# cp2k/dbcsr

Measured on AMD Instinct MI355X. Metric: block-sparse multiply GFLOP/s (fp64), higher is better.
Workload: dtype f64; 1 GPU; config2_32768_23x23_fill10_fp64; M=32768, c_nblks=2030625, nproducts=29207882, k_passes=1, parallelism=1 GPU

## Files before the change

dbcsr_amd/csrc/mm_exact.h:

```cpp
#ifndef DBCSR_AMD_MM_EXACT_H
#define DBCSR_AMD_MM_EXACT_H
#include "mm_types.h"
#include "smm_core.h"
#include "mm_epilogue.h"

#ifndef DBCSR_EXACT_ALL_PIECES
#define DBCSR_EXACT_ALL_PIECES 1
#endif
#ifndef DBCSR_EXACT_SCHED_BARRIER
#define DBCSR_EXACT_SCHED_BARRIER 1
#endif

namespace dbcsr_amd {

template <int LD>
struct Pitch {
  static constexpr int PAD = (LD % 16 == 0) ? 2 : 0;
  static constexpr int P = LD + PAD;
};

constexpr int cmax(int a, int b) { return a > b ? a : b; }
template <int V>
struct IntC {
  static constexpr int value = V;
};

constexpr int class_wave_lds(int m, int n, int k0, int k1, int k2) {
  int a_lds = 0, cb_max = 0, bpad = 0;
  const int ks[3] = {k0, k1, k2};
  for (int i = 0; i < 3; ++i) {
    const int k = ks[i];
    if (k <= 0) continue;
    const int k4 = 4 * ((k + 3) / 4), ap = m + ((m % 16 == 0) ? 2 : 0);
    a_lds = cmax(a_lds, ap * k4 * 8);
    cb_max = cmax(cb_max, (k * n * 8 + 1023) / 1024);
    if (k % 16 == 0) bpad = 128;
  }
  a_lds = (a_lds + 15) & ~15;
  const int c_lds = ((m * n * 8 + 1023) / 1024) * 1024;
  return (cmax(a_lds + cb_max * (1024 + bpad) + 16, c_lds) + 15) & ~15;
}

template <int M, int N, int K>
struct KShape {
  static constexpr int KS = (K + 3) / 4, K4 = 4 * KS;
  static constexpr int AP = Pitch<M>::P, BP = Pitch<K>::P;
  static constexpr int A_LDS = AP * K4 * 8, B_LDS = BP * N * 8;
  static constexpr int CA = (M * K4 * 8 + 1023) / 1024, CB = (K * N * 8 + 1023) / 1024;
};
template <int M, int N>
struct KShape<M, N, 0> {
  static constexpr int KS = 0, K4 = 0, AP = 0, BP = 0, A_LDS = 0, B_LDS = 0, CA = 0, CB = 0;
};

template <int M, int N, int K0, int K1, int K2>
struct ClassShape {
  static constexpr int MA = (M + 7) / 8, NC = (N + 7) / 8;
  static constexpr int A_LDS = (cmax(KShape<M, N, K0>::A_LDS, cmax(KShape<M, N, K1>::A_LDS, KShape<M, N, K2>::A_LDS)) + 15) & ~15;
  static constexpr int CAMAX = cmax(KShape<M, N, K0>::CA, cmax(KShape<M, N, K1>::CA, KShape<M, N, K2>::CA));
  static constexpr int CBMAX = cmax(KShape<M, N, K0>::CB, cmax(KShape<M, N, K1>::CB, KShape<M, N, K2>::CB));
  static constexpr int BPAD = ((K0 % 16 == 0) || (K1 != 0 && K1 % 16 == 0) || (K2 != 0 && K2 % 16 == 0)) ? 128 : 0;
  static constexpr int B_REGION = CBMAX * (1024 + BPAD) + 16;
  static constexpr int C_LDS = ((M * N * 8 + 1023) / 1024) * 1024;
  static constexpr int WAVE_LDS = (cmax(A_LDS + B_REGION, C_LDS) + 15) & ~15;
  static_assert(WAVE_LDS == class_wave_lds(M, N, K0, K1, K2), "host and device disagree on the LDS size of a class");
};

template <int LD>
__device__ __forceinline__ int staged_offset(int c, int lane) {
  if constexpr (Pitch<LD>::PAD == 0)
    return c * 1024 + lane * 16;
  else
    return c * 1024 + lane * 16 + Pitch<LD>::PAD * 8 * ((c * 128) / LD + (lane * 2) / LD);
}

template <int M, int N, int K0, int K1, int K2>
__device__ __forceinline__ void cblock_f64_classes(const Desc& d, const Entry first, bool have_first, const Entry* __restrict__ entries,
                                                   const double* __restrict__ a_data,
                                                   const double* __restrict__ b_data, double* __restrict__ c_out,
                                                   const double* __restrict__ c_in, double alpha, double beta, const LaneMap& L, int lane,
                                                   char* lds, double* __restrict__ norm_out, double drop_below = 0.0) {
  typedef ClassShape<M, N, K0, K1, K2> CS;
  constexpr int MA = CS::MA, NC = CS::NC;
  constexpr int AP = Pitch<M>::P;
  char* lds_a = lds;
  char* lds_b = lds + CS::A_LDS;
  double acc[MA][NC];
#pragma unroll
  for (int a = 0; a < MA; ++a)
#pragma unroll
    for (int c = 0; c < NC; ++c) acc[a][c] = 0.0;
  const Entry* e = entries + d.prod_start;
  const int cnt = d.prod_cnt;
  const int voff = lane * 16;
  u32x4 ra[CS::CAMAX], rb[CS::CBMAX];

  const double* pa[MA];
  int colc[NC];
#pragma unroll
  for (int a = 0; a < MA; ++a) {
    int row = 8 * a + L.rowl;
    row = row < M ? row : M - 1;
    pa[a] = reinterpret_cast<const double*>(lds_a) + row + AP * L.kq;
  }
#pragma unroll
  for (int c = 0; c < NC; ++c) {
    int col = 8 * c + L.coll;
    colc[c] = col < N ? col : N - 1;
  }

  int ebase = 0;
  uint32_t ev0 = 0, ev1 = 0, ev2 = 1;
  auto load_window = [&](int base) {
    ebase = base;
    if (cnt <= 0) return;
    const int i = base + lane < cnt ? base + lane : cnt - 1;
    ev0 = e[i].a_lo;
    ev1 = e[i].b_lo;
    ev2 = e[i].w;
  };
  load_window(0);
  auto entry_at = [&](int i) {
    if (i - ebase >= 64) load_window(i);
    const int j = __builtin_amdgcn_readfirstlane(i - ebase);
    Entry en;
    en.a_lo = (uint32_t)__builtin_amdgcn_readlane((int)ev0, j);
    en.b_lo = (uint32_t)__builtin_amdgcn_readlane((int)ev1, j);
    en.w = (uint32_t)__builtin_amdgcn_readlane((int)ev2, j);
    return en;
  };
  auto in_set = [](int ks) { return ks == K0 || (K1 != 0 && ks == K1) || (K2 != 0 && ks == K2); };
  auto next_in_set = [&](int i) {
    while (i < cnt && !in_set(entry_at(i).ks())) ++i;
    return i;
  };

  auto issue = [&](const Entry& en) {
    const int ks = en.ks();
    const int abytes = __builtin_amdgcn_readfirstlane(M * ks * 8), bbytes = __builtin_amdgcn_readfirstlane(ks * N * 8);
    const int nca = __builtin_amdgcn_readfirstlane((M * ((ks + 3) & ~3) * 8 + 1023) >> 10), ncb = (bbytes + 1023) >> 10;
    const __amdgpu_buffer_rsrc_t rsa = __builtin_amdgcn_make_buffer_rsrc((void*)(a_data + en.a_off()), 0, abytes, 0x00020000);
    const __amdgpu_buffer_rsrc_t rsb = __builtin_amdgcn_make_buffer_rsrc((void*)(b_data + en.b_off()), 0, bbytes, 0x00020000);
#pragma unroll
    for (int c = 0; c < CS::CAMAX; ++c)
      if (DBCSR_EXACT_ALL_PIECES || c < nca) ra[c] = __builtin_amdgcn_raw_buffer_load_b128(rsa, voff, c * 1024, 0);
#pragma unroll
    for (int c = 0; c < CS::CBMAX; ++c)
      if (DBCSR_EXACT_ALL_PIECES || c < ncb) rb[c] = __builtin_amdgcn_raw_buffer_load_b128(rsb, voff, c * 1024, 0);
  };
  auto store = [&](int ks) {
    const int nca = __builtin_amdgcn_readfirstlane((M * ((ks + 3) & ~3) * 8 + 1023) >> 10);
    const int ncb = __builtin_amdgcn_readfirstlane((ks * N * 8 + 1023) >> 10);
#pragma unroll
    for (int c = 0; c < CS::CAMAX; ++c)
      if (DBCSR_EXACT_ALL_PIECES || c < nca) *reinterpret_cast<u32x4*>(lds_a + staged_offset<M>(c, lane)) = ra[c];
    DBCSR_AMD_LDS_ORDER();
    const int sh = __builtin_amdgcn_readfirstlane((ks & 15) == 0 ? (ks == 16 ? 4 : 5) : 31);
#pragma unroll
    for (int c = 0; c < CS::CBMAX; ++c)
      if (DBCSR_EXACT_ALL_PIECES || c < ncb) *reinterpret_cast<u32x4*>(lds_b + c * 1024 + lane * 16 + 16 * ((c * 128 + lane * 2) >> sh)) = rb[c];
  };
  auto compute_k = [&](auto kc) {
    constexpr int K = decltype(kc)::value;
    typedef KShape<M, N, K> KSH;
    constexpr int KS = KSH::KS, BP = KSH::BP;
    const double* pb[NC];
    const double* pbt[NC];
#pragma unroll
    for (int c = 0; c < NC; ++c) {
      pb[c] = reinterpret_cast<const double*>(lds_b) + L.kq + BP * colc[c];
      const int kt = 4 * (KS - 1) + L.kq;
      pbt[c] = reinterpret_cast<const double*>(lds_b) + (kt < K ? kt : 0) + BP * colc[c];
    }
    const bool tail_in = 4 * (KS - 1) + L.kq < K;
    double av[2][MA], bv[2][NC];
    auto fetch = [&](int s, int buf) {
#pragma unroll
      for (int a = 0; a < MA; ++a) av[buf][a] = pa[a][s * 4 * AP];
#pragma unroll
      for (int c = 0; c < NC; ++c) bv[buf][c] = (s == KS - 1 && (K & 3)) ? (tail_in ? pbt[c][0] : 0.0) : pb[c][4 * s];
    };
    fetch(0, 0);
#pragma unroll
    for (int s = 0; s < KS; ++s) {
      if (s + 1 < KS) fetch(s + 1, (s + 1) & 1);
#pragma unroll
      for (int a = 0; a < MA; ++a)
#pragma unroll
        for (int c = 0; c < NC; ++c) acc[a][c] = __builtin_amdgcn_mfma_f64_4x4x4f64(av[s & 1][a], bv[s & 1][c], acc[a][c], 0, 0, 0);
      if (DBCSR_EXACT_SCHED_BARRIER) __builtin_amdgcn_sched_barrier(0);
    }
  };

  int i0;
  Entry e0;
  if (have_first && in_set(first.ks())) {
    i0 = 0;
    e0 = first;
    issue(e0);
  } else {
    i0 = next_in_set(0);
    e0 = i0 < cnt ? entry_at(i0) : Entry::make(0, 0, K0);
    if (i0 < cnt) issue(e0);
  }
  while (i0 < cnt) {
    const int kcur = e0.ks();
    const int i1 = next_in_set(i0 + 1);
    const Entry e1 = i1 < cnt ? entry_at(i1) : e0;
    store(kcur);
    if (i1 < cnt) issue(e1);
    if (kcur == K0) compute_k(IntC<K0>());
    if constexpr (K1 != 0)
      if (kcur == K1) compute_k(IntC<K1>());
    if constexpr (K2 != 0)
      if (kcur == K2) compute_k(IntC<K2>());
    i0 = i1;
    e0 = e1;
  }
  for (int p = 0; p < cnt; ++p) {
    const Entry ep = e[p];
    if (!in_set(ep.ks())) block_product_f64<MA, NC, false>(acc, a_data + ep.a_off(), b_data + ep.b_off(), M, N, ep.ks(), L);
  }

  const bool has_in = d.cin_off >= 0;
  if (norm_out && drop_below > 0.0 && !has_in) {
    const double s2 = acc_norm2<M, N>(acc, alpha, L);
    if (lane == 0) *norm_out = s2;
    if (s2 < drop_below) return;
    norm_out = nullptr;
  }
  stage_c_block<M, N>(reinterpret_cast<double*>(lds), acc, alpha, L);
  store_c_block<M, N>(lds, c_out + d.c_off, has_in ? c_in + d.cin_off : nullptr, beta, lane, norm_out);
}

template <int M, int N, int K0, int K1, int K2>
__device__ __forceinline__ void mm_class_kernel_body(const Desc* __restrict__ descs, int64_t nblk, const Entry* __restrict__ entries,
                                                     const double* __restrict__ a_data, const double* __restrict__ b_data,
                                                     double* __restrict__ c_out, const double* __restrict__ c_in, double alpha, double beta,
                                                     int skip_empty, const int* __restrict__ order, const Work* __restrict__ work,
                                                     double* __restrict__ norms, char* smem) {
  const int lane = threadIdx.x & 63;
  const int wid = __builtin_amdgcn_readfirstlane((int)(threadIdx.x >> 6));
  const int wg = xcd_remap(blockIdx.x, gridDim.x);
  const int64_t pos = (int64_t)wg * (int)(blockDim.x >> 6) + wid;
  Desc d;
  Entry first = Entry::make(0, 0, 0);
  bool have_first = false;
  int64_t cbi = 0;
  if (work) {
    const Work w = work[pos];
    if (w.prod_cnt < 0) return;
    cbi = w.cb;
    d.c_off = w.c_off, d.cin_off = w.cin_off, d.prod_start = w.prod_start, d.prod_cnt = w.prod_cnt, d.m = w.m, d.n = w.n;
    first.a_lo = w.a_lo, first.b_lo = w.b_lo, first.w = w.w;
    have_first = w.prod_cnt > 0;
  } else {
    const int64_t cb = order[pos];
    if (cb < 0 || cb >= nblk) return;
    d = descs[cb];
    cbi = cb;
  }
  const double drop_below = norms ? norms[nblk] : 0.0;
  if (skip_empty && d.prod_cnt == 0) return;
  const LaneMap L(lane);
  cblock_f64_classes<M, N, K0, K1, K2>(d, first, have_first, entries, a_data, b_data, c_out, c_in, alpha, beta, L, lane,
                                       smem + (size_t)wid * ClassShape<M, N, K0, K1, K2>::WAVE_LDS, norms ? norms + cbi : nullptr, drop_below);
}


template <int M, int N, int K0, int K1, int K2, int G>
__device__ __forceinline__ void mm_class_stream_body(const Desc* __restrict__ descs, int64_t nblk, const Entry* __restrict__ entries,
                                                     const double* __restrict__ a_data, const double* __restrict__ b_data,
                                                     double* __restrict__ c_out, const double* __restrict__ c_in, double alpha, double beta,
                                                     int skip_empty, const int* __restrict__ order, char* smem) {
  static_assert(G >= 1 && G <= 64, "one lane per block of the group");
  typedef ClassShape<M, N, K0, K1, K2> CS;
  constexpr int MA = CS::MA, NC = CS::NC;
  constexpr int AP = Pitch<M>::P;
  const int lane = threadIdx.x & 63;
  const int wid = __builtin_amdgcn_readfirstlane((int)(threadIdx.x >> 6));
  const int wg = xcd_remap(blockIdx.x, gridDim.x);
  const int64_t pos0 = ((int64_t)wg * 4 + wid) * G;
  char* lds = smem + (size_t)wid * CS::WAVE_LDS;
  char* lds_a = lds;
  char* lds_b = lds + CS::A_LDS;
  const LaneMap L(lane);
  const int voff = lane * 16;

  const int my_cb = lane < G ? order[pos0 + lane] : -1;
  const bool my_ok = my_cb >= 0 && my_cb < nblk;
  const Desc my_d = descs[my_ok ? my_cb : 0];
  const int my_cnt = my_ok ? my_d.prod_cnt : -1;
  auto lane_i32 = [&](int v, int l) { return __builtin_amdgcn_readlane(v, l); };
  auto lane_i64 = [&](int64_t v, int l) {
    const uint32_t lo = (uint32_t)__builtin_amdgcn_readlane((int)(uint32_t)v, l);
    const uint32_t hi = (uint32_t)__builtin_amdgcn_readlane((int)(uint32_t)((uint64_t)v >> 32), l);
    return (int64_t)(((uint64_t)hi << 32) | lo);
  };

  const double* pa[MA];
  int colc[NC];
#pragma unroll
  for (int a = 0; a < MA; ++a) {
    int row = 8 * a + L.rowl;
    row = row < M ? row : M - 1;
    pa[a] = reinterpret_cast<const double*>(lds_a) + row + AP * L.kq;
  }
#pragma unroll
  for (int c = 0; c < NC; ++c) {
    int col = 8 * c + L.coll;
    colc[c] = col < N ? col : N - 1;
  }
  u32x4 ra[CS::CAMAX], rb[CS::CBMAX];
  double acc[MA][NC];

  uint32_t w0[2] = {0, 0}, w1[2] = {0, 0}, w2[2] = {1, 1};
  auto load_window = [&](int buf, int b) {
    const int cnt = lane_i32(my_cnt, b);
    if (cnt <= 0) return;
    const Entry* e = entries + lane_i64(my_d.prod_start, b);
    const int i = lane < cnt ? lane : cnt - 1;
    const uint32_t x0 = e[i].a_lo, x1 = e[i].b_lo, x2 = e[i].w;
    if (buf) {
      w0[1] = x0, w1[1] = x1, w2[1] = x2;
    } else {
      w0[0] = x0, w1[0] = x1, w2[0] = x2;
    }
  };
  auto entry_at = [&](int buf, int b, int i) {
    Entry en;
    if (i < 64) {
      en.a_lo = (uint32_t)__builtin_amdgcn_readlane((int)(buf ? w0[1] : w0[0]), i);
      en.b_lo = (uint32_t)__builtin_amdgcn_readlane((int)(buf ? w1[1] : w1[0]), i);
      en.w = (uint32_t)__builtin_amdgcn_readlane((int)(buf ? w2[1] : w2[0]), i);
    } else {
      en = entries[lane_i64(my_d.prod_start, b) + i];
    }
    return en;
  };
  auto in_set = [](int ks) { return ks == K0 || (K1 != 0 && ks == K1) || (K2 != 0 && ks == K2); };

  auto issue = [&](const Entry& en) {
    const int ks = en.ks();
    const int abytes = __builtin_amdgcn_readfirstlane(M * ks * 8), bbytes = __builtin_amdgcn_readfirstlane(ks * N * 8);
    const __amdgpu_buffer_rsrc_t rsa = __builtin_amdgcn_make_buffer_rsrc((void*)(a_data + en.a_off()), 0, abytes, 0x00020000);
    const __amdgpu_buffer_rsrc_t rsb = __builtin_amdgcn_make_buffer_rsrc((void*)(b_data + en.b_off()), 0, bbytes, 0x00020000);
#pragma unroll
    for (int c = 0; c < CS::CAMAX; ++c) ra[c] = __builtin_amdgcn_raw_buffer_load_b128(rsa, voff, c * 1024, 0);
#pragma unroll
    for (int c = 0; c < CS::CBMAX; ++c) rb[c] = __builtin_amdgcn_raw_buffer_load_b128(rsb, voff, c * 1024, 0);
  };
  auto store = [&](int ks) {
#pragma unroll
    for (int c = 0; c < CS::CAMAX; ++c) *reinterpret_cast<u32x4*>(lds_a + staged_offset<M>(c, lane)) = ra[c];
    DBCSR_AMD_LDS_ORDER();
    const int sh = __builtin_amdgcn_readfirstlane((ks & 15) == 0 ? (ks == 16 ? 4 : 5) : 31);
#pragma unroll
    for (int c = 0; c < CS::CBMAX; ++c) *reinterpret_cast<u32x4*>(lds_b + c * 1024 + lane * 16 + 16 * ((c * 128 + lane * 2) >> sh)) = rb[c];
  };
  auto compute_k = [&](auto kc) {
    constexpr int K = decltype(kc)::value;
    typedef KShape<M, N, K> KSH;
    constexpr int KS = KSH::KS, BP = KSH::BP;
    const double* pb[NC];
    const double* pbt[NC];
#pragma unroll
    for (int c = 0; c < NC; ++c) {
      pb[c] = reinterpret_cast<const double*>(lds_b) + L.kq + BP * colc[c];
      const int kt = 4 * (KS - 1) + L.kq;
      pbt[c] = reinterpret_cast<const double*>(lds_b) + (kt < K ? kt : 0) + BP * colc[c];
    }
    const bool tail_in = 4 * (KS - 1) + L.kq < K;
    double av[2][MA], bv[2][NC];
    auto fetch = [&](int s, int buf) {
#pragma unroll
      for (int a = 0; a < MA; ++a) av[buf][a] = pa[a][s * 4 * AP];
#pragma unroll
      for (int c = 0; c < NC; ++c) bv[buf][c] = (s == KS - 1 && (K & 3)) ? (tail_in ? pbt[c][0] : 0.0) : pb[c][4 * s];
    };
    fetch(0, 0);
#pragma unroll
    for (int s = 0; s < KS; ++s) {
      if (s + 1 < KS) fetch(s + 1, (s + 1) & 1);
#pragma unroll
      for (int a = 0; a < MA; ++a)
#pragma unroll
        for (int c = 0; c < NC; ++c) acc[a][c] = __builtin_amdgcn_mfma_f64_4x4x4f64(av[s & 1][a], bv[s & 1][c], acc[a][c], 0, 0, 0);
      if (DBCSR_EXACT_SCHED_BARRIER) __builtin_amdgcn_sched_barrier(0);
    }
  };

  auto block_cnt = [&](int b) { return b < G ? lane_i32(my_cnt, b) : -1; };
  auto first_in_set = [&](int buf, int b, int from) {
    const int cnt = block_cnt(b);
    int i = from;
    while (i < cnt && !in_set(entry_at(buf, b, i).ks())) ++i;
    return i < cnt ? i : -1;
  };

  load_window(0, 0);
  int nb = 0, ni = first_in_set(0, 0, 0);
  bool in_flight = false;
  Entry ne = Entry::make(0, 0, K0);
  if (ni >= 0) {
    ne = entry_at(0, 0, ni);
    issue(ne);
    in_flight = true;
  }
  for (int b = 0; b < G; ++b) {
    const int buf = b & 1;
    const int cnt = block_cnt(b);
    if (b + 1 < G) load_window(buf ^ 1, b + 1);
    if (cnt < 0 || (skip_empty && cnt == 0)) {
      if (!in_flight && b + 1 < G) {
        ni = first_in_set(buf ^ 1, b + 1, 0);
        nb = b + 1;
        if (ni >= 0) {
          ne = entry_at(buf ^ 1, b + 1, ni);
          issue(ne);
          in_flight = true;
        }
      }
      continue;
    }
#pragma unroll
    for (int a = 0; a < MA; ++a)
#pragma unroll
      for (int c = 0; c < NC; ++c) acc[a][c] = 0.0;
    while (in_flight && nb == b) {
      const int kcur = ne.ks();
      store(kcur);
      int i1 = first_in_set(buf, b, ni + 1);
      in_flight = false;
      if (i1 >= 0) {
        ni = i1;
        ne = entry_at(buf, b, i1);
        issue(ne);
        in_flight = true;
      } else if (b + 1 < G) {
        i1 = first_in_set(buf ^ 1, b + 1, 0);
        nb = b + 1;
        ni = i1;
        if (i1 >= 0) {
          ne = entry_at(buf ^ 1, b + 1, i1);
          issue(ne);
          in_flight = true;
        }
      }
      if (kcur == K0) compute_k(IntC<K0>());
      if constexpr (K1 != 0)
        if (kcur == K1) compute_k(IntC<K1>());
      if constexpr (K2 != 0)
        if (kcur == K2) compute_k(IntC<K2>());
    }
    if (!in_flight && nb <= b && b + 1 < G) {
      ni = first_in_set(buf ^ 1, b + 1, 0);
      nb = b + 1;
      if (ni >= 0) {
        ne = entry_at(buf ^ 1, b + 1, ni);
        issue(ne);
        in_flight = true;
      }
    }
    const int64_t d_c_off = lane_i64(my_d.c_off, b), d_cin_off = lane_i64(my_d.cin_off, b), d_ps = lane_i64(my_d.prod_start, b);
    for (int p = 0; p < cnt; ++p) {
      const Entry ep = entries[d_ps + p];
      if (!in_set(ep.ks())) block_product_f64<MA, NC, false>(acc, a_data + ep.a_off(), b_data + ep.b_off(), M, N, ep.ks(), L);
    }
    stage_c_block<M, N>(reinterpret_cast<double*>(lds), acc, alpha, L);
    store_c_block<M, N>(lds, c_out + d_c_off, d_cin_off >= 0 ? c_in + d_cin_off : nullptr, beta, lane, nullptr);
  }
}

}

#ifdef DBCSR_AMD_JIT_M
#ifndef DBCSR_AMD_JIT_MINW
#define DBCSR_AMD_JIT_MINW 1
#endif
extern "C" __global__ void __launch_bounds__(256, DBCSR_AMD_JIT_MINW)
    mm_numeric_f64_class(const dbcsr_amd::Desc* __restrict__ descs, long nblk, const dbcsr_amd::Entry* __restrict__ entries,
                         const double* __restrict__ a_data, const double* __restrict__ b_data, double* __restrict__ c_out,
                         const double* __restrict__ c_in, double alpha, double beta, int skip_empty, const int* __restrict__ order,
                         const dbcsr_amd::Work* __restrict__ work, double* __restrict__ norms) {
  extern __shared__ __attribute__((aligned(16))) char smem[];
#if defined(DBCSR_AMD_JIT_G) && DBCSR_AMD_JIT_G > 1
  dbcsr_amd::mm_class_stream_body<DBCSR_AMD_JIT_M, DBCSR_AMD_JIT_N, DBCSR_AMD_JIT_K0, DBCSR_AMD_JIT_K1, DBCSR_AMD_JIT_K2, DBCSR_AMD_JIT_G>(
      descs, nblk, entries, a_data, b_data, c_out, c_in, alpha, beta, skip_empty, order, smem);
#else
  dbcsr_amd::mm_class_kernel_body<DBCSR_AMD_JIT_M, DBCSR_AMD_JIT_N, DBCSR_AMD_JIT_K0, DBCSR_AMD_JIT_K1, DBCSR_AMD_JIT_K2>(
      descs, nblk, entries, a_data, b_data, c_out, c_in, alpha, beta, skip_empty, order, work, norms, smem);
#endif
}
#endif
#endif
```

dbcsr_amd/csrc/mm_jit.hip:

```cpp
#include "mm_jit.h"

#include <dlfcn.h>
#include <unistd.h>
#include <cstdint>

#include <cstdio>
#include <cstdlib>
#include <cstring>
#include <map>
#include <mutex>
#include <string>
#include <tuple>
#include <vector>

#include "mm_exact.h"
#include "smm_exact.h"

namespace dbcsr_amd {
namespace {

#include "jit_sources.inc"

typedef struct _hiprtcProgram* rtc_program;
struct Rtc {
  void* lib = nullptr;
  int (*CreateProgram)(rtc_program*, const char*, const char*, int, const char**, const char**) = nullptr;
  int (*CompileProgram)(rtc_program, int, const char**) = nullptr;
  int (*GetProgramLogSize)(rtc_program, size_t*) = nullptr;
  int (*GetProgramLog)(rtc_program, char*) = nullptr;
  int (*GetCodeSize)(rtc_program, size_t*) = nullptr;
  int (*GetCode)(rtc_program, char*) = nullptr;
  int (*DestroyProgram)(rtc_program*) = nullptr;
  int (*Version)(int*, int*) = nullptr;
  bool ok = false;
};

Rtc& rtc() {
  static Rtc r;
  static std::once_flag once;
  std::call_once(once, [] {
    for (const char* name : {"libhiprtc.so", "libhiprtc.so.7", "/opt/rocm/lib/libhiprtc.so"}) {
      r.lib = dlopen(name, RTLD_NOW | RTLD_GLOBAL);
      if (r.lib) break;
    }
    if (!r.lib) {
      fprintf(stderr, "dbcsr_amd: cannot load libhiprtc (%s): mixed block sizes run the generic kernels\n", dlerror());
      return;
    }
#define DBCSR_SYM(field, sym)                               \
  *reinterpret_cast<void**>(&r.field) = dlsym(r.lib, sym);  \
  if (!r.field) return;
    DBCSR_SYM(CreateProgram, "hiprtcCreateProgram")
    DBCSR_SYM(CompileProgram, "hiprtcCompileProgram")
    DBCSR_SYM(GetProgramLogSize, "hiprtcGetProgramLogSize")
    DBCSR_SYM(GetProgramLog, "hiprtcGetProgramLog")
    DBCSR_SYM(GetCodeSize, "hiprtcGetCodeSize")
    DBCSR_SYM(GetCode, "hiprtcGetCode")
    DBCSR_SYM(DestroyProgram, "hiprtcDestroyProgram")
#undef DBCSR_SYM
    *reinterpret_cast<void**>(&r.Version) = dlsym(r.lib, "hiprtcVersion");
    r.ok = true;
  });
  return r;
}

struct Cached {
  std::vector<char> image;
  hipModule_t mod = nullptr;
  ClassKernel k;
  bool failed = false;
};
std::mutex g_mu;
std::map<std::tuple<int, int, int, int, int, int, int>, Cached> g_cache;

bool g_last_from_cache = false;
int compile_and_load(const char* defs, const char* tu_name, const char* what, const char* entry, const hipDeviceProp_t& prop, hipModule_t* mod,
                     hipFunction_t* fn, size_t* code_size, std::vector<char>* image) {
  Rtc& r = rtc();
  if (!r.ok) return -1;
  g_last_from_cache = false;
  const char* hsrc[] = {kJitSrc_mm_types, kJitSrc_smm_core, kJitSrc_mm_epilogue, kJitSrc_mm_exact, kJitSrc_smm_exact};
  const char* hname[] = {"mm_types.h", "smm_core.h", "mm_epilogue.h", "mm_exact.h", "smm_exact.h"};
  rtc_program prog = nullptr;
  if (r.CreateProgram(&prog, defs, tu_name, (int)(sizeof hname / sizeof hname[0]), hsrc, hname) != 0) return -1;
  std::string arch = std::string("--offload-arch=") + prop.gcnArchName;
  std::vector<std::string> extra;
  if (const char* d = getenv("DBCSR_AMD_JIT_DEFS")) {
    std::string all(d);
    size_t pos = 0;
    while (pos < all.size()) {
      const size_t e = all.find(' ', pos);
      const std::string tok = all.substr(pos, e == std::string::npos ? std::string::npos : e - pos);
      if (!tok.empty()) extra.push_back(tok);
      if (e == std::string::npos) break;
      pos = e + 1;
    }
  }
  std::vector<const char*> opts = {arch.c_str(), "-O3", "-std=c++17", "-munsafe-fp-atomics"};
  for (const std::string& t : extra) opts.push_back(t.c_str());
  std::string cache_file;
  if (const char* dir = getenv("DBCSR_AMD_JIT_CACHE")) {
    if (*dir) {
      uint64_t h = 1469598103934665603ull;
      auto mix = [&h](const char* t) {
        for (; *t; ++t) h = (h ^ (unsigned char)*t) * 1099511628211ull;
        h = (h ^ 0xffu) * 1099511628211ull;
      };
      mix(defs);
      for (const char* t : hsrc) mix(t);
      for (const char* t : opts) mix(t);
      int vmaj = 0, vmin = 0;
      if (r.Version) r.Version(&vmaj, &vmin);
      char tail[64];
      snprintf(tail, sizeof tail, "hiprtc %d.%d entry %s", vmaj, vmin, entry);
      mix(tail);
      char name[40];
      snprintf(name, sizeof name, "/dbcsr_amd_%016llx.co", (unsigned long long)h);
      cache_file = std::string(dir) + name;
      if (FILE* f = fopen(cache_file.c_str(), "rb")) {
        std::vector<char>& code = *image;
        code.clear();
        char buf[65536];
        size_t got;
        while ((got = fread(buf, 1, sizeof buf, f)) > 0) code.insert(code.end(), buf, buf + got);
        fclose(f);
        bool sound = false;
        if (code.size() > 24) {
          uint64_t head[3];
          memcpy(head, code.data(), 24);
          if (head[0] == 0x314f435f444d4143ull && head[1] == code.size() - 24) {
            uint64_t ph = 1469598103934665603ull;
            for (size_t i = 24; i < code.size(); ++i) ph = (ph ^ (unsigned char)code[i]) * 1099511628211ull;
            sound = ph == head[2];
          }
        }
        if (sound) code.erase(code.begin(), code.begin() + 24);
        if (sound && hipModuleLoadData(mod, code.data()) == hipSuccess) {
          if (hipModuleGetFunction(fn, *mod, entry) == hipSuccess) {
            r.DestroyProgram(&prog);
            if (code_size) *code_size = code.size();
            g_last_from_cache = true;
            if (getenv("DBCSR_AMD_MM_VERBOSE")) fprintf(stderr, "dbcsr_amd: %s from %s\n", what, cache_file.c_str());
            return 0;
          }
          (void)hipModuleUnload(*mod);
        }
        (void)hipGetLastError();
      }
    }
  }
  const int rc = r.CompileProgram(prog, (int)opts.size(), opts.data());
  if (rc != 0) {
    size_t ls = 0;
    r.GetProgramLogSize(prog, &ls);
    std::string log(ls + 1, 0);
    if (ls) r.GetProgramLog(prog, &log[0]);
    fprintf(stderr, "dbcsr_amd: hiprtc failed for %s:\n%s\n", what, log.c_str());
    r.DestroyProgram(&prog);
    return -1;
  }
  size_t cs = 0;
  r.GetCodeSize(prog, &cs);
  std::vector<char>& code = *image;
  code.assign(cs, 0);
  r.GetCode(prog, code.data());
  r.DestroyProgram(&prog);
  if (!cache_file.empty()) {
    const std::string tmp = cache_file + "." + std::to_string((long)getpid()) + ".tmp";
    if (FILE* f = fopen(tmp.c_str(), "wb")) {
      uint64_t head[3] = {0x314f435f444d4143ull, (uint64_t)code.size(), 1469598103934665603ull};
      for (char ch : code) head[2] = (head[2] ^ (unsigned char)ch) * 1099511628211ull;
      const bool ok = fwrite(head, 1, 24, f) == 24 && fwrite(code.data(), 1, code.size(), f) == code.size();
      if (fclose(f) != 0 || !ok || rename(tmp.c_str(), cache_file.c_str()) != 0) remove(tmp.c_str());
    }
  }
  if (hipModuleLoadData(mod, code.data()) != hipSuccess) return -1;
  if (hipModuleGetFunction(fn, *mod, entry) != hipSuccess) return -1;
  if (code_size) *code_size = cs;
  return 0;
}

struct CachedStack {
  std::vector<char> image;
  hipModule_t mod = nullptr;
  StackKernel k;
  bool failed = false;
};
std::map<std::tuple<int, int, int, int, int>, CachedStack> g_stack_cache;

}

int jit_class_kernel(int m, int n, int k0, int k1, int k2, int g, ClassKernel* out) {
  if (g < 1 || g > 64) return -1;
  if (!out || m < 1 || n < 1 || k0 < 1 || m > 32 || n > 32 || k0 > 32 || k1 > 32 || k2 > 32) return -1;
  int dev = 0;
  if (hipGetDevice(&dev) != hipSuccess) return -1;
  std::lock_guard<std::mutex> lock(g_mu);
  auto key = std::make_tuple(dev, m, n, k0, k1, k2, g);
  auto it = g_cache.find(key);
  if (it != g_cache.end()) {
    if (it->second.failed) return -1;
    *out = it->second.k;
    return 0;
  }
  Cached& c = g_cache[key];
  c.failed = true;
  hipDeviceProp_t prop;
  if (hipGetDeviceProperties(&prop, dev) != hipSuccess) return -1;
  const int wave_lds = class_wave_lds(m, n, k0, k1, k2);
  int wgs = (160 * 1024) / (4 * wave_lds);
  int minw = wgs > 4 ? 4 : (wgs < 1 ? 1 : wgs);
  if (g > 1 && minw > 1) --minw;
  char defs[512];
  snprintf(defs, sizeof defs,
           "#define DBCSR_AMD_JIT_M %d\n#define DBCSR_AMD_JIT_N %d\n#define DBCSR_AMD_JIT_K0 %d\n#define DBCSR_AMD_JIT_K1 %d\n"
           "#define DBCSR_AMD_JIT_K2 %d\n#define DBCSR_AMD_JIT_MINW %d\n#define DBCSR_AMD_JIT_G %d\n#include \"mm_exact.h\"\n",
           m, n, k0, k1, k2, minw, g);
  char what[96];
  snprintf(what, sizeof what, "class (%d, %d; %d, %d, %d)", m, n, k0, k1, k2);
  size_t cs = 0;
  if (compile_and_load(defs, "mm_class.hip", what, "mm_numeric_f64_class", prop, &c.mod, &c.k.fn, &cs, &c.image) != 0) return -1;
  c.k.wave_lds = wave_lds;
  c.failed = false;
  if (getenv("DBCSR_AMD_MM_VERBOSE") && !g_last_from_cache) fprintf(stderr, "dbcsr_amd: compiled class kernel (%d, %d; %d, %d, %d), %zu bytes, %d B LDS per wave\n", m, n, k0, k1, k2, cs, wave_lds);
  *out = c.k;
  return 0;
}


int jit_stack_kernel(int m, int n, int k, bool bt, StackKernel* out, bool compile) {
  if (!out || m < 1 || n < 1 || k < 1 || m > 32 || n > 32 || k > 32) return -1;
  int dev = 0;
  if (hipGetDevice(&dev) != hipSuccess) return -1;
  std::lock_guard<std::mutex> lock(g_mu);
  auto key = std::make_tuple(dev, m, n, k, (int)bt);
  auto it = g_stack_cache.find(key);
  if (it != g_stack_cache.end()) {
    if (it->second.failed) return -1;
    *out = it->second.k;
    return 0;
  }
  if (!compile) return 1;
  CachedStack& c = g_stack_cache[key];
  c.failed = true;
  hipDeviceProp_t prop;
  if (hipGetDeviceProperties(&prop, dev) != hipSuccess) return -1;
  const int wave_lds = stack_wave_lds(m, n, k, bt);
  int wgs = (160 * 1024) / (4 * wave_lds);
  const int minw = wgs > 4 ? 4 : (wgs < 1 ? 1 : wgs);
  char defs[512];
  snprintf(defs, sizeof defs,
           "#define DBCSR_AMD_JIT_SM %d\n#define DBCSR_AMD_JIT_SN %d\n#define DBCSR_AMD_JIT_SK %d\n#define DBCSR_AMD_JIT_SBT %d\n"
           "#define DBCSR_AMD_JIT_MINW %d\n#include \"smm_exact.h\"\n",
           m, n, k, bt ? 1 : 0, minw);
  char what[96];
  snprintf(what, sizeof what, "stack kernel (%d, %d, %d%s)", m, n, k, bt ? "; B transposed" : "");
  size_t cs = 0;
  if (compile_and_load(defs, "smm_stack_exact.hip", what, "smm_stack_f64_exact", prop, &c.mod, &c.k.fn, &cs, &c.image) != 0) return -1;
  c.k.wave_lds = wave_lds;
  c.failed = false;
  if (getenv("DBCSR_AMD_MM_VERBOSE") && !g_last_from_cache) fprintf(stderr, "dbcsr_amd: compiled %s, %zu bytes, %d B LDS per wave\n", what, cs, wave_lds);
  *out = c.k;
  return 0;
}

}
```

Baseline: 37360 GFLOP/s.

## Shrink per-wave LDS to the exact B image and guard staging stores

The per-wave LDS budget for each class now uses the padded B image size instead of whole 1 KiB pieces plus pad. Smaller LDS per wave allows more waves per CU. Staging stores are now skipped for pieces past the real A/B image, and are masked per lane when a piece would run past the smaller region. The JIT cache key now includes DBCSR_AMD_JIT_DEFS. The shared LDS-size helper moves into its own header that is also passed to the JIT compiler. The risk is extra branching in the store path and possible LDS overlap if the bounds logic is wrong.

```diff
diff --git a/dbcsr_amd/csrc/mm_class_lds.h b/dbcsr_amd/csrc/mm_class_lds.h
--- /dev/null
+++ b/dbcsr_amd/csrc/mm_class_lds.h
@@ -0,0 +1,24 @@
+#ifndef DBCSR_AMD_MM_CLASS_LDS_H
+#define DBCSR_AMD_MM_CLASS_LDS_H
+
+namespace dbcsr_amd {
+
+constexpr int cmax(int a, int b) { return a > b ? a : b; }
+
+constexpr int class_wave_lds(int m, int n, int k0, int k1, int k2) {
+  int a_lds = 0, b_lds = 0;
+  const int ks[3] = {k0, k1, k2};
+  for (int i = 0; i < 3; ++i) {
+    const int k = ks[i];
+    if (k <= 0) continue;
+    const int k4 = 4 * ((k + 3) / 4), ap = m + ((m % 16 == 0) ? 2 : 0), bp = k + ((k % 16 == 0) ? 2 : 0);
+    a_lds = cmax(a_lds, ap * k4 * 8);
+    b_lds = cmax(b_lds, (bp * n * 8 + 15) & ~15);
+  }
+  a_lds = (a_lds + 15) & ~15;
+  const int c_lds = ((m * n * 8 + 1023) / 1024) * 1024;
+  return (cmax(a_lds + b_lds, c_lds) + 15) & ~15;
+}
+
+}
+#endif
diff --git a/dbcsr_amd/csrc/mm_exact.h b/dbcsr_amd/csrc/mm_exact.h
--- a/dbcsr_amd/csrc/mm_exact.h
+++ b/dbcsr_amd/csrc/mm_exact.h
@@ -3,6 +3,7 @@
 #include "mm_types.h"
 #include "smm_core.h"
 #include "mm_epilogue.h"
+#include "mm_class_lds.h"
 
 #ifndef DBCSR_EXACT_ALL_PIECES
 #define DBCSR_EXACT_ALL_PIECES 1
@@ -19,33 +20,16 @@
   static constexpr int P = LD + PAD;
 };
 
-constexpr int cmax(int a, int b) { return a > b ? a : b; }
 template <int V>
 struct IntC {
   static constexpr int value = V;
 };
 
-constexpr int class_wave_lds(int m, int n, int k0, int k1, int k2) {
-  int a_lds = 0, cb_max = 0, bpad = 0;
-  const int ks[3] = {k0, k1, k2};
-  for (int i = 0; i < 3; ++i) {
-    const int k = ks[i];
-    if (k <= 0) continue;
-    const int k4 = 4 * ((k + 3) / 4), ap = m + ((m % 16 == 0) ? 2 : 0);
-    a_lds = cmax(a_lds, ap * k4 * 8);
-    cb_max = cmax(cb_max, (k * n * 8 + 1023) / 1024);
-    if (k % 16 == 0) bpad = 128;
-  }
-  a_lds = (a_lds + 15) & ~15;
-  const int c_lds = ((m * n * 8 + 1023) / 1024) * 1024;
-  return (cmax(a_lds + cb_max * (1024 + bpad) + 16, c_lds) + 15) & ~15;
-}
-
 template <int M, int N, int K>
 struct KShape {
   static constexpr int KS = (K + 3) / 4, K4 = 4 * KS;
   static constexpr int AP = Pitch<M>::P, BP = Pitch<K>::P;
-  static constexpr int A_LDS = AP * K4 * 8, B_LDS = BP * N * 8;
+  static constexpr int A_LDS = AP * K4 * 8, B_LDS = (BP * N * 8 + 15) & ~15;
   static constexpr int CA = (M * K4 * 8 + 1023) / 1024, CB = (K * N * 8 + 1023) / 1024;
 };
 template <int M, int N>
@@ -59,11 +43,13 @@
   static constexpr int A_LDS = (cmax(KShape<M, N, K0>::A_LDS, cmax(KShape<M, N, K1>::A_LDS, KShape<M, N, K2>::A_LDS)) + 15) & ~15;
   static constexpr int CAMAX = cmax(KShape<M, N, K0>::CA, cmax(KShape<M, N, K1>::CA, KShape<M, N, K2>::CA));
   static constexpr int CBMAX = cmax(KShape<M, N, K0>::CB, cmax(KShape<M, N, K1>::CB, KShape<M, N, K2>::CB));
-  static constexpr int BPAD = ((K0 % 16 == 0) || (K1 != 0 && K1 % 16 == 0) || (K2 != 0 && K2 % 16 == 0)) ? 128 : 0;
-  static constexpr int B_REGION = CBMAX * (1024 + BPAD) + 16;
+  static constexpr int B_LDS = cmax(KShape<M, N, K0>::B_LDS, cmax(KShape<M, N, K1>::B_LDS, KShape<M, N, K2>::B_LDS));
   static constexpr int C_LDS = ((M * N * 8 + 1023) / 1024) * 1024;
-  static constexpr int WAVE_LDS = (cmax(A_LDS + B_REGION, C_LDS) + 15) & ~15;
+  static constexpr int WAVE_LDS = (cmax(A_LDS + B_LDS, C_LDS) + 15) & ~15;
   static_assert(WAVE_LDS == class_wave_lds(M, N, K0, K1, K2), "host and device disagree on the LDS size of a class");
+  static constexpr bool B_PADDED = (K0 % 16 == 0) || (K1 != 0 && K1 % 16 == 0) || (K2 != 0 && K2 % 16 == 0);
+  static constexpr bool a_piece_passes(int c) { return c * 1024 + 1024 + (Pitch<M>::PAD ? 16 * ((c * 128 + 126) / M) : 0) > WAVE_LDS; }
+  static constexpr bool b_piece_passes(int c) { return A_LDS + c * 1024 + 1024 + (B_PADDED ? 16 * ((c * 128 + 126) / 16) : 0) > WAVE_LDS; }
 };
 
 template <int LD>
@@ -72,6 +58,25 @@
     return c * 1024 + lane * 16;
   else
     return c * 1024 + lane * 16 + Pitch<LD>::PAD * 8 * ((c * 128) / LD + (lane * 2) / LD);
+}
+
+template <class CS, int M, int N>
+__device__ __forceinline__ void stage_pieces(char* lds_a, char* lds_b, const u32x4 (&ra)[CS::CAMAX], const u32x4 (&rb)[CS::CBMAX], int ks, int lane) {
+  const int voff = lane * 16;
+  const int aimg = __builtin_amdgcn_readfirstlane(M * ((ks + 3) & ~3) * 8), bimg = __builtin_amdgcn_readfirstlane(ks * N * 8);
+#pragma unroll
+  for (int c = 0; c < CS::CAMAX; ++c)
+    if (c * 1024 < aimg) {
+      if (!CS::a_piece_passes(c) || c * 1024 + voff < aimg) *reinterpret_cast<u32x4*>(lds_a + staged_offset<M>(c, lane)) = ra[c];
+    }
+  DBCSR_AMD_LDS_ORDER();
+  const int sh = __builtin_amdgcn_readfirstlane((ks & 15) == 0 ? (ks == 16 ? 4 : 5) : 31);
+#pragma unroll
+  for (int c = 0; c < CS::CBMAX; ++c)
+    if (c * 1024 < bimg) {
+      if (!CS::b_piece_passes(c) || c * 1024 + voff < bimg)
+        *reinterpret_cast<u32x4*>(lds_b + c * 1024 + lane * 16 + 16 * ((c * 128 + lane * 2) >> sh)) = rb[c];
+    }
 }
 
 template <int M, int N, int K0, int K1, int K2>
@@ -148,18 +153,7 @@
     for (int c = 0; c < CS::CBMAX; ++c)
       if (DBCSR_EXACT_ALL_PIECES || c < ncb) rb[c] = __builtin_amdgcn_raw_buffer_load_b128(rsb, voff, c * 1024, 0);
   };
-  auto store = [&](int ks) {
-    const int nca = __builtin_amdgcn_readfirstlane((M * ((ks + 3) & ~3) * 8 + 1023) >> 10);
-    const int ncb = __builtin_amdgcn_readfirstlane((ks * N * 8 + 1023) >> 10);
-#pragma unroll
-    for (int c = 0; c < CS::CAMAX; ++c)
-      if (DBCSR_EXACT_ALL_PIECES || c < nca) *reinterpret_cast<u32x4*>(lds_a + staged_offset<M>(c, lane)) = ra[c];
-    DBCSR_AMD_LDS_ORDER();
-    const int sh = __builtin_amdgcn_readfirstlane((ks & 15) == 0 ? (ks == 16 ? 4 : 5) : 31);
-#pragma unroll
-    for (int c = 0; c < CS::CBMAX; ++c)
-      if (DBCSR_EXACT_ALL_PIECES || c < ncb) *reinterpret_cast<u32x4*>(lds_b + c * 1024 + lane * 16 + 16 * ((c * 128 + lane * 2) >> sh)) = rb[c];
-  };
+  auto store = [&](int ks) { stage_pieces<CS, M, N>(lds_a, lds_b, ra, rb, ks, lane); };
   auto compute_k = [&](auto kc) {
     constexpr int K = decltype(kc)::value;
     typedef KShape<M, N, K> KSH;
@@ -350,14 +344,7 @@
 #pragma unroll
     for (int c = 0; c < CS::CBMAX; ++c) rb[c] = __builtin_amdgcn_raw_buffer_load_b128(rsb, voff, c * 1024, 0);
   };
-  auto store = [&](int ks) {
-#pragma unroll
-    for (int c = 0; c < CS::CAMAX; ++c) *reinterpret_cast<u32x4*>(lds_a + staged_offset<M>(c, lane)) = ra[c];
-    DBCSR_AMD_LDS_ORDER();
-    const int sh = __builtin_amdgcn_readfirstlane((ks & 15) == 0 ? (ks == 16 ? 4 : 5) : 31);
-#pragma unroll
-    for (int c = 0; c < CS::CBMAX; ++c) *reinterpret_cast<u32x4*>(lds_b + c * 1024 + lane * 16 + 16 * ((c * 128 + lane * 2) >> sh)) = rb[c];
-  };
+  auto store = [&](int ks) { stage_pieces<CS, M, N>(lds_a, lds_b, ra, rb, ks, lane); };
   auto compute_k = [&](auto kc) {
     constexpr int K = decltype(kc)::value;
     typedef KShape<M, N, K> KSH;
diff --git a/dbcsr_amd/csrc/mm_jit.hip b/dbcsr_amd/csrc/mm_jit.hip
--- a/dbcsr_amd/csrc/mm_jit.hip
+++ b/dbcsr_amd/csrc/mm_jit.hip
@@ -71,7 +71,7 @@
   bool failed = false;
 };
 std::mutex g_mu;
-std::map<std::tuple<int, int, int, int, int, int, int>, Cached> g_cache;
+std::map<std::tuple<int, int, int, int, int, int, int, std::string>, Cached> g_cache;
 
 bool g_last_from_cache = false;
 int compile_and_load(const char* defs, const char* tu_name, const char* what, const char* entry, const hipDeviceProp_t& prop, hipModule_t* mod,
@@ -79,8 +79,8 @@
   Rtc& r = rtc();
   if (!r.ok) return -1;
   g_last_from_cache = false;
-  const char* hsrc[] = {kJitSrc_mm_types, kJitSrc_smm_core, kJitSrc_mm_epilogue, kJitSrc_mm_exact, kJitSrc_smm_exact};
-  const char* hname[] = {"mm_types.h", "smm_core.h", "mm_epilogue.h", "mm_exact.h", "smm_exact.h"};
+  const char* hsrc[] = {kJitSrc_mm_types, kJitSrc_smm_core, kJitSrc_mm_epilogue, kJitSrc_mm_class_lds, kJitSrc_mm_exact, kJitSrc_smm_exact};
+  const char* hname[] = {"mm_types.h", "smm_core.h", "mm_epilogue.h", "mm_class_lds.h", "mm_exact.h", "smm_exact.h"};
   rtc_program prog = nullptr;
   if (r.CreateProgram(&prog, defs, tu_name, (int)(sizeof hname / sizeof hname[0]), hsrc, hname) != 0) return -1;
   std::string arch = std::string("--offload-arch=") + prop.gcnArchName;
@@ -196,7 +196,8 @@
   int dev = 0;
   if (hipGetDevice(&dev) != hipSuccess) return -1;
   std::lock_guard<std::mutex> lock(g_mu);
-  auto key = std::make_tuple(dev, m, n, k0, k1, k2, g);
+  const char* jit_defs = getenv("DBCSR_AMD_JIT_DEFS");
+  auto key = std::make_tuple(dev, m, n, k0, k1, k2, g, std::string(jit_defs ? jit_defs : ""));
   auto it = g_cache.find(key);
   if (it != g_cache.end()) {
     if (it->second.failed) return -1;
```

Result: no change. 37390 GFLOP/s, median of 5 (+0.1%).
